# JaronTu/Multimodal_MVD_Seg

Measured on AMD Instinct MI355X. Metric: train-step samples/sec on 4-modality 128^3 patches (PlainConvUNet 3d_fullres, fp32), higher is better.
Workload: dtype f32; 1 GPU; BASELINE configs[1]: PlainConvUNet 3d_fullres 6 stages 31.2M params, 4x128x128x128 patch, 5 classes, fp32, DC+CE deep supervision, SGD-Nesterov+clip; per_gpu_batch=2, global_batch=2, parallelism=dp1, step_launch=one hipGraph replay per step (captured after 3 eager steps)

## Files before the change

include/mvdseg_hip.h:

```cpp
#ifndef MVDSEG_HIP_H
#define MVDSEG_HIP_H
#include <stddef.h>
#include <stdint.h>

#ifdef __cplusplus
extern "C" {
#endif

#define MVD_VERSION 100
#define MVD_MAX_TAPS 27

int mvd_version(void);
const char *mvd_last_error(void);
int mvd_has_mfma(void);
int mvd_set_conv_engine(int mode);
int mvd_set_wino_min_items(long n);

int mvd_pack_weight(const float *w, float *wf, float *wb, int K, int C, int T, int transposed, void *stream);

size_t mvd_conv_fwd_workspace_bytes(int N, long out_voxels, int K);
int mvd_conv3d_fwd(const float *x1, int C1, const float *x2, int C2, const float *wf, const float *bias, float *y,
                   int N, int D, int H, int W, int K, const int ksize[3], const int stride[3], void *ws,
                   size_t ws_bytes, void *stream);
int mvd_conv3d_dgrad(const float *dy, const float *wb, float *dx1, int C1, float *dx2, int C2, int N, int D, int H,
// ... 52 lines not shown
                                const int *C, const int *T, const int *transposed, void *stream);
int mvd_pack_weights_bf16_batch_pad(int n, const float *const *w, uint16_t *const *wf, uint16_t *const *wb, const int *K,
                                    const int *C, const int *T, const int *transposed, const int *Csrc, void *stream);
int mvd_conv3d_fwd_bf16(const uint16_t *x1, int C1, const uint16_t *x2, int C2, const uint16_t *wf, const float *bias,
                        uint16_t *y, int N, int D, int H, int W, int K, const int ksize[3], const int stride[3],
                        void *ws, size_t ws_bytes, void *stream);
int mvd_conv3d_dgrad_bf16(const uint16_t *dy, const uint16_t *wb, uint16_t *dx1, int C1, uint16_t *dx2, int C2, int N,
                          int D, int H, int W, int K, const int ksize[3], const int stride[3], void *ws, size_t ws_bytes,
                          void *stream);
int mvd_convT3d_fwd_bf16(const uint16_t *x, const uint16_t *wf, const float *bias, uint16_t *y, int N, int D, int H, int W,
                         int C, int K, const int stride[3], void *ws, size_t ws_bytes, void *stream);
int mvd_convT3d_dgrad_bf16(const uint16_t *dy, const uint16_t *wb, uint16_t *dx, int N, int D, int H, int W, int C, int K,
                           const int stride[3], void *ws, size_t ws_bytes, void *stream);
int mvd_conv3d_wgrad_bf16(const uint16_t *x1, int C1, const uint16_t *x2, int C2, const uint16_t *dy, float *dw,
                          float *dbias, int N, int D, int H, int W, int K, const int ksize[3], const int stride[3],
                          void *ws, size_t ws_bytes, void *stream);
int mvd_convT3d_wgrad_bf16(const uint16_t *x, const uint16_t *dy, float *dw, float *dbias, int N, int D, int H, int W,
                           int C, int K, const int stride[3], void *ws, size_t ws_bytes, void *stream);
int mvd_conv3d_fwd_bf16_stats_tiles(int N, int D, int H, int W, int C1, int C2, int K, const int ksize[3],
                                    const int stride[3]);
int mvd_conv3d_dgrad_acc_ok(int is_bf16, int N, int D, int H, int W, int C1, int K, const int ksize[3], const int stride[3]);
int mvd_conv3d_dgrad_acc(const float *dy, const float *wb, float *dx1, int C1, int N, int D, int H, int W, int K,
                         const int ksize[3], const int stride[3], void *stream);
int mvd_conv3d_dgrad_bf16_acc(const uint16_t *dy, const uint16_t *wb, uint16_t *dx1, int C1, int N, int D, int H, int W, int K,
                              const int ksize[3], const int stride[3], void *ws, size_t ws_bytes, void *stream);
int mvd_set_bf16_zmarch_kernel(int which);
int mvd_set_bf16_wgrad_kernel(int which);
int mvd_conv3d_wgrad_bf16_prologue_ok(int N, int D, int H, int W, int C1, int C2, int K, const int ksize[3], const int stride[3]);
int mvd_conv3d_wgrad_bf16_fused(const uint16_t *x1, int C1, const uint16_t *dy, float *dw, float *dbias, int N, int D, int H, int W,
                                int K, const int ksize[3], const int stride[3], const float *in_scale, const float *in_shift,
                                float slope, void *ws, size_t ws_bytes, void *stream);
int mvd_conv3d_fwd_bf16_prologue_ok(int N, int D, int H, int W, int C1, int C2, int K, const int ksize[3],
                                    const int stride[3]);
int mvd_conv3d_fwd_bf16_fused(const uint16_t *x1, int C1, const uint16_t *x2, int C2, const uint16_t *wf, const float *bias,
                              uint16_t *y, int N, int D, int H, int W, int K, const int ksize[3], const int stride[3],
                              const float *in_scale, const float *in_shift, float slope, float *tile_stats, int *ntiles_out,
                              void *ws, size_t ws_bytes, void *stream);
int mvd_instnorm_finalize_tiles(const float *tile_stats, long ntiles, const float *gamma, const float *beta, float *mean,
                                float *rstd, float *scale, float *shift, int N, long V, int C, float eps, void *stream);
int mvd_instnorm_lrelu_apply_bf16(const uint16_t *x, const float *scale, const float *shift, uint16_t *y, int N, long V,
                                  int C, float slope, void *stream);
int mvd_instnorm_stats_bf16(const void *x, int x_is_bf16, const float *gamma, const float *beta, float *mean, float *rstd,
                            float *scale, float *shift, int N, long V, int C, float eps, void *ws, size_t ws_bytes,
                            void *stream);
int mvd_instnorm_lrelu_fwd_bf16(const void *x, int x_is_bf16, const float *gamma, const float *beta, uint16_t *y,
                                float *mean, float *rstd, int N, long V, int C, float eps, float slope, void *ws,
// ... 281 lines not shown
```

multimodal_mvd_seg_amd/_lib.py:

```python
import ctypes
import os
from ctypes import c_double, c_float, c_int, c_long, c_size_t, c_uint64, c_void_p

_HERE = os.path.dirname(os.path.abspath(__file__))
LIB_PATH = os.path.join(_HERE, "libmvdseg_hip.so")

_P = c_void_p
_I3 = ctypes.c_int * 3

CONV_DIRECT, CONV_WINO2, CONV_WINO3, CONV_WINO2P = 0, 1, 2, 3

SIGNATURES = {
    "mvd_version": (c_int, []),
    "mvd_last_error": (ctypes.c_char_p, []),
    "mvd_has_mfma": (c_int, []),
    "mvd_set_conv_engine": (c_int, [c_int]),
    "mvd_set_wino_min_items": (c_int, [c_long]),
    "mvd_pack_weight": (c_int, [_P, _P, _P, c_int, c_int, c_int, c_int, _P]),
    "mvd_conv_fwd_workspace_bytes": (c_size_t, [c_int, c_long, c_int]),
    "mvd_conv3d_fwd": (c_int, [_P, c_int, _P, c_int, _P, _P, _P, c_int, c_int, c_int, c_int, c_int, _I3, _I3, _P,
                               c_size_t, _P]),
    "mvd_conv3d_dgrad": (c_int, [_P, _P, _P, c_int, _P, c_int, c_int, c_int, c_int, c_int, c_int, _I3, _I3, _P,
                                 c_size_t, _P]),
    "mvd_conv3d_wgrad_workspace_bytes": (c_size_t, [c_int, c_int, c_int, c_int, c_int, c_int, c_int]),
# ... 20 lines not shown
    "mvd_conv_wino3_applicable": (c_int, [c_int, c_int, c_int, c_int, c_int, c_int, c_int, _I3, _I3]),
    "mvd_wino3_weight_elems": (c_size_t, [c_int, c_int]),
    "mvd_pack_weight_wino3": (c_int, [_P, _P, _P, c_int, c_int, _P]),
    "mvd_pack_weights_batch3": (c_int, [c_int] + [_P] * 11 + [_P]),
    "mvd_set_wino2p_min_items": (c_int, [c_long]),
    "mvd_conv_wino2p_applicable": (c_int, [c_int, c_int, c_int, c_int, c_int, c_int, c_int, _I3, _I3]),
    "mvd_wino2p_weight_elems": (c_size_t, [c_int, c_int]),
    "mvd_pack_weight_wino2p": (c_int, [_P, _P, _P, c_int, c_int, _P]),
    "mvd_set_wgrad_wino3_min_items": (c_int, [c_long]),
    "mvd_conv_wgrad_wino3_applicable": (c_int, [c_int, c_int, c_int, c_int, c_int, c_int, c_int, _I3, _I3]),
    "mvd_wgrad_wino3_launches": (c_long, []),
    "mvd_set_wgrad_bias_fold": (c_int, [c_int]),
    "mvd_conv3d_wgrad_bf16": (c_int, [_P, c_int, _P, c_int, _P, _P, _P, c_int, c_int, c_int, c_int, c_int, _I3, _I3, _P,
                                      c_size_t, _P]),
    "mvd_convT3d_wgrad_bf16": (c_int, [_P, _P, _P, _P, c_int, c_int, c_int, c_int, c_int, c_int, _I3, _P, c_size_t,
                                       _P]),
    "mvd_instnorm_lrelu_fwd_prestats": (c_int, [_P, _P, c_long, _P, _P, _P, _P, _P, c_int, c_long, c_int, c_float, c_float,
                                                _P, c_size_t, _P]),
    "mvd_conv3d_fwd_bf16_stats_tiles": (c_int, [c_int, c_int, c_int, c_int, c_int, c_int, c_int, _I3, _I3]),
    "mvd_set_bf16_zmarch_kernel": (c_int, [c_int]),
    "mvd_set_bf16_wgrad_kernel": (c_int, [c_int]),
    "mvd_conv3d_dgrad_acc_ok": (c_int, [c_int, c_int, c_int, c_int, c_int, c_int, c_int, _I3, _I3]),
    "mvd_conv3d_dgrad_acc": (c_int, [_P, _P, _P, c_int, c_int, c_int, c_int, c_int, c_int, _I3, _I3, _P]),
    "mvd_conv3d_dgrad_bf16_acc": (c_int, [_P, _P, _P, c_int, c_int, c_int, c_int, c_int, c_int, _I3, _I3, _P, c_size_t, _P]),
    "mvd_conv3d_fwd_bf16_prologue_ok": (c_int, [c_int, c_int, c_int, c_int, c_int, c_int, c_int, _I3, _I3]),
    "mvd_conv3d_wgrad_bf16_prologue_ok": (c_int, [c_int, c_int, c_int, c_int, c_int, c_int, c_int, _I3, _I3]),
    "mvd_conv3d_wgrad_bf16_fused": (c_int, [_P, c_int, _P, _P, _P, c_int, c_int, c_int, c_int, c_int, _I3, _I3, _P, _P, c_float,
                                            _P, c_size_t, _P]),
    "mvd_instnorm_stats_bf16": (c_int, [_P, c_int, _P, _P, _P, _P, _P, _P, c_int, c_long, c_int, c_float, _P, c_size_t, _P]),
    "mvd_conv3d_fwd_bf16_fused": (c_int, [_P, c_int, _P, c_int, _P, _P, _P, c_int, c_int, c_int, c_int, c_int, _I3, _I3, _P,
                                          _P, c_float, _P, _P, _P, c_size_t, _P]),
    "mvd_instnorm_finalize_tiles": (c_int, [_P, c_long, _P, _P, _P, _P, _P, _P, c_int, c_long, c_int, c_float, _P]),
    "mvd_instnorm_lrelu_apply_bf16": (c_int, [_P, _P, _P, _P, c_int, c_long, c_int, c_float, _P]),
    "mvd_instnorm_lrelu_fwd_bf16": (c_int, [_P, c_int, _P, _P, _P, _P, _P, c_int, c_long, c_int, c_float, c_float, _P,
                                            c_size_t, _P]),
    "mvd_instnorm_lrelu_bwd_bf16": (c_int, [_P, c_int, _P, _P, _P, _P, _P, _P, _P, _P, c_int, c_long, c_int, c_float, _P,
                                            c_size_t, _P]),
    "mvd_seghead_fwd_bf16": (c_int, [_P, _P, _P, _P, c_int, c_long, c_int, c_int, _P]),
    "mvd_seghead_bwd_bf16": (c_int, [_P, _P, _P, _P, _P, _P, c_int, c_long, c_int, c_int, c_int, _P, c_size_t, _P]),
    "mvd_seghead_bf16_fused_ok": (c_int, [c_int, c_long, c_int, c_int]),
    "mvd_seghead_fwd_fused": (c_int, [_P, _P, _P, _P, _P, c_float, _P, _P, _P, c_int, c_long, c_int, c_int, _P]),
    "mvd_seghead_bwd_fused": (c_int, [_P, _P, _P, _P, _P, c_float, _P, _P, _P, _P, _P, c_int, c_long, c_int, c_int, c_int, _P,
                                      c_size_t, _P]),
    "mvd_instnorm_stats_from_tiles": (c_int, [_P, c_long, _P, _P, c_int, c_long, c_int, c_float, _P, c_size_t, _P]),
    "mvd_seghead_fwd_bf16_fused": (c_int, [_P, _P, _P, c_float, _P, _P, _P, c_int, c_long, c_int, c_int, _P]),
    "mvd_seghead_bwd_bf16_fused": (c_int, [_P, _P, _P, c_float, _P, _P, _P, _P, _P, c_int, c_long, c_int, c_int, c_int, _P,
# ... 180 lines not shown
```

multimodal_mvd_seg_amd/csrc/conv.hip:

```cpp
#include "common.h"
#include "conv_geom.h"

namespace mvd {

static int g_engine_mode = 0;
#define g_wino_off (wino_mode() == 0)
static const int g_transp_off = getenv("MVD_TRANSP") ? (atoi(getenv("MVD_TRANSP")) == 0) : 0;
static long g_wino_min_items = getenv("MVD_WINO_MIN") ? atol(getenv("MVD_WINO_MIN")) : 256;
static const long kWino3MinItemsDefault = 128;
static long g_wino3_min_items = getenv("MVD_WINO3_MIN") ? atol(getenv("MVD_WINO3_MIN")) : kWino3MinItemsDefault;
static const long kWino2pMinItemsDefault = 256;
static long g_wino2p_min_items = getenv("MVD_WINO2P_MIN") ? atol(getenv("MVD_WINO2P_MIN")) : kWino2pMinItemsDefault;

struct ConvPass {
    int N, D, H, W, R1, R2, P1, P2;
    const int *ks, *st;
};
static ConvPass fwd_pass(int N, int D, int H, int W, int C1, int C2, int K, const int ks[3], const int st[3]) {
    return {N, D, H, W, C1, C2, K, 0, ks, st};
}
static ConvPass dgrad_pass(int N, int D, int H, int W, int C1, int C2, int K, const int ks[3], const int st[3]) {
    return {N, D, H, W, K, 0, C1, C2, ks, st};
}
static bool wino_pass_ok(const ConvPass &p, int kd) {
// ... 462 lines not shown
        if (uf[q] || ub[q] || vf[q] || vb[q])
            MVD_REQUIRE((T[q] == 27 || (T[q] == 9 && !vf[q] && !vb[q])) && !transposed[q] && K[q] % 32 == 0 && C[q] % 32 == 0,
                        "pack_weights_batch3: Winograd tables need a 3x3x3 (or, uf / ub, 1x3x3) conv with C %% 32 == 0 and K %% 32 == 0");
    }
    return pack_weights_batch(n, w, wf, wb, uf, ub, K, C, T, transposed, as_stream(stream), vf, vb);
}

int mvd_set_wino2p_min_items(long n) {
    g_wino2p_min_items = n < 0 ? kWino2pMinItemsDefault : n;
    return 0;
}

size_t mvd_wino2p_weight_elems(int C, int K) { return (size_t)16 * C * K; }

int mvd_pack_weight_wino2p(const float *w, float *uf, float *ub, int K, int C, void *stream) {
    MVD_REQUIRE(w && (uf || ub) && K > 0 && C > 0, "pack_weight_wino2p: bad arguments");
    MVD_REQUIRE(K % 32 == 0 && C % 32 == 0, "pack_weight_wino2p: needs C %% 32 == 0 and K %% 32 == 0");
    return pack_weight_wino2p(w, uf, ub, K, C, as_stream(stream));
}

static bool k3s2(const int ks[3], const int st[3]) {
    return ks[0] == 3 && ks[1] == 3 && ks[2] == 3 && st[0] == 2 && st[1] == 2 && st[2] == 2;
}
static const long kDgrad32sMinVoxels = 4096;
static bool dgrad32s_eligible(int N, int D, int H, int W, int C2, const int ks[3], const int st[3]) {
    static const int dg2 = getenv("MVD_DGRAD2") ? atoi(getenv("MVD_DGRAD2")) : 1;
    if (!dg2 || g_engine_mode != 0 || C2 != 0 || !k3s2(ks, st)) return false;
    return (long)N * conv_out_dim(D, 3, 2) * conv_out_dim(H, 3, 2) * conv_out_dim(W, 3, 2) >= kDgrad32sMinVoxels || g_wino_min_items <= 1;
}

int mvd_conv3d_dgrad_routed(const float *dy, const float *wb, const float *table, int table_kind, float *dx1, int C1, float *dx2,
                            int C2, int N, int D, int H, int W, int K, const int ksize[3], const int stride[3], void *ws,
                            size_t ws_bytes, void *stream) {
    MVD_REQUIRE(dy && wb && dx1 && C1 > 0 && C2 >= 0 && (C2 == 0 || dx2), "conv3d_dgrad: null pointer / bad channels");
    MVD_REQUIRE(N > 0 && D > 0 && H > 0 && W > 0 && K > 0, "conv3d_dgrad: bad shape");
    if (check_ks(ksize, stride, "conv3d_dgrad")) return 2;
    MVD_REQUIRE(table_kind >= MVD_CONV_DIRECT && table_kind <= MVD_CONV_WINO2P, "conv3d_dgrad: unknown table kind");
    MVD_REQUIRE(!(table && table_kind == MVD_CONV_WINO2P) || (ksize[0] == 1 && ksize[1] == 3 && ksize[2] == 3),
                "conv3d_dgrad: the in-plane table is that of a 1x3x3 kernel");
    if (dgrad32s_eligible(N, D, H, W, C2, ksize, stride)) {
        int r = dgrad32s(N, D, H, W, C1, K, conv_out_dim(D, 3, 2), conv_out_dim(H, 3, 2), conv_out_dim(W, 3, 2), dy, wb, dx1,
                         as_stream(stream));
        if (r >= 0) return r;
    }
    const WinoTable tab = {table, table_kind, ksize, stride};
    for (int pd = 0; pd < stride[0]; pd++)
        for (int ph = 0; ph < stride[1]; ph++)
            for (int pw = 0; pw < stride[2]; pw++) {
                const int p[3] = {pd, ph, pw};
                FwdGeom g;
                if (!conv_dgrad_class_geom(g, N, D, H, W, C1, C2, K, ksize, stride, p)) continue;
                int r = run_fwd(g, dy, nullptr, wb, nullptr, dx1, dx2, ws, ws_bytes, as_stream(stream), &tab);
                if (r) return r;
            }
    return 0;
}

int mvd_conv3d_dgrad(const float *dy, const float *wb, float *dx1, int C1, float *dx2, int C2, int N, int D, int H, int W,
                     int K, const int ksize[3], const int stride[3], void *ws, size_t ws_bytes, void *stream) {
    return mvd_conv3d_dgrad_routed(dy, wb, nullptr, MVD_CONV_DIRECT, dx1, C1, dx2, C2, N, D, H, W, K, ksize, stride, ws, ws_bytes,
                                   stream);
}

size_t mvd_conv3d_wgrad_workspace_bytes(int C, int K, int T, int N, int Do, int Ho, int Wo) {
    WgradGeom g;
    memset(&g, 0, sizeof(g));
    g.N = N; g.Do = Do; g.Ho = Ho; g.Wo = Wo; g.C1 = C; g.C2 = 0; g.K = K; g.ntaps = g.T = T;
    size_t a = max_sz(wgrad_scalar_ws(g), wgrad_mfma_ws(g));
    return max_sz(a, colsum_ws((long)N * Do * Ho * Wo, K));
}

int mvd_set_wgrad_wino3_min_items(long n) {
    set_wgrad_wino3_min_items(n);
    return 0;
}

int mvd_conv_wgrad_wino3_applicable(int N, int D, int H, int W, int C1, int C2, int K, const int ksize[3],
// ... 206 lines not shown
                const int p[3] = {pd, ph, pw};
                FwdGeom g;
                if (!conv_dgrad_class_geom(g, N, D, H, W, C1, C2, K, ksize, stride, p)) continue;
                g.acc = (int8_t)acc;
                int r = run_fwd16(g, dy, nullptr, wb, nullptr, dx1, dx2, ws, ws_bytes, as_stream(stream));
                if (r) return r;
            }
    return 0;
}

int mvd_conv3d_dgrad_bf16(const uint16_t *dy, const uint16_t *wb, uint16_t *dx1, int C1, uint16_t *dx2, int C2, int N, int D, int H, int W,
                     int K, const int ksize[3], const int stride[3], void *ws, size_t ws_bytes, void *stream) {
    return dgrad_bf16_impl(dy, wb, dx1, C1, dx2, C2, N, D, H, W, K, ksize, stride, ws, ws_bytes, stream, 0);
}

static bool strided3(const int ksize[3], const int stride[3]) {
    return ksize[0] == 3 && ksize[1] == 3 && ksize[2] == 3 && (stride[0] == 2 || stride[1] == 2 || stride[2] == 2);
}

int mvd_conv3d_dgrad_acc_ok(int is_bf16, int N, int D, int H, int W, int C1, int K, const int ksize[3], const int stride[3]) {
    if (!conv_args_ok(N, D, H, W, C1, 0, K, ksize, stride, "conv3d_dgrad_acc_ok")) return 0;
    if (C1 % 32 || K % 32 || g_engine_mode != 0) return 0;
    if (is_bf16) return strided3(ksize, stride) ? 1 : 0;
    return (dgrad32s_eligible(N, D, H, W, 0, ksize, stride) &&
            (long)conv_out_dim(D, 3, 2) * conv_out_dim(H, 3, 2) * conv_out_dim(W, 3, 2) * K * 4 < (1L << 31)) ? 1 : 0;
}

int mvd_conv3d_dgrad_bf16_acc(const uint16_t *dy, const uint16_t *wb, uint16_t *dx1, int C1, int N, int D, int H, int W, int K,
                              const int ksize[3], const int stride[3], void *ws, size_t ws_bytes, void *stream) {
    MVD_REQUIRE(mvd_conv3d_dgrad_acc_ok(1, N, D, H, W, C1, K, ksize, stride), "conv3d_dgrad_bf16_acc: no accumulating kernel for this "
                "shape (ask mvd_conv3d_dgrad_acc_ok first)");
    return dgrad_bf16_impl(dy, wb, dx1, C1, nullptr, 0, N, D, H, W, K, ksize, stride, ws, ws_bytes, stream, 1);
}

int mvd_conv3d_dgrad_acc(const float *dy, const float *wb, float *dx1, int C1, int N, int D, int H, int W, int K,
                         const int ksize[3], const int stride[3], void *stream) {
    MVD_REQUIRE(dy && wb && dx1, "conv3d_dgrad_acc: null pointer");
    MVD_REQUIRE(mvd_conv3d_dgrad_acc_ok(0, N, D, H, W, C1, K, ksize, stride), "conv3d_dgrad_acc: no accumulating kernel for this shape "
                "(ask mvd_conv3d_dgrad_acc_ok first)");
    int r = dgrad32s(N, D, H, W, C1, K, conv_out_dim(D, 3, 2), conv_out_dim(H, 3, 2), conv_out_dim(W, 3, 2), dy, wb, dx1, as_stream(stream), 1);
    if (r < 0) {
        set_error("conv3d_dgrad_acc: the fused stride-2 kernel refused the shape");
        return 3;
    }
    return r;
}

int mvd_convT3d_fwd_bf16(const uint16_t *x, const uint16_t *wf, const float *bias, uint16_t *y, int N, int D, int H, int W, int C, int K,
                    const int stride[3], void *ws, size_t ws_bytes, void *stream) {
    MVD_REQUIRE(x && wf && y && N > 0 && D > 0 && H > 0 && W > 0 && C > 0 && K > 0, "convT3d_fwd_bf16: bad arguments");
    for (int a = 0; a < 3; a++) MVD_REQUIRE(stride[a] == 1 || stride[a] == 2, "convT3d_fwd_bf16: stride must be 1 or 2");
    if (!g_transp_off) {
        int r = convT_fwd_direct16(x, wf, bias, y, N, D, H, W, C, K, stride, as_stream(stream));
        if (r >= 0) return r;
    }
    for (int pd = 0; pd < stride[0]; pd++)
        for (int ph = 0; ph < stride[1]; ph++)
            for (int pw = 0; pw < stride[2]; pw++) {
                const int p[3] = {pd, ph, pw};
                FwdGeom g;
                convT_fwd_class_geom(g, N, D, H, W, C, K, stride, p);
                int r = run_fwd16(g, x, nullptr, wf, bias, y, nullptr, ws, ws_bytes, as_stream(stream));
                if (r) return r;
            }
    return 0;
}

int mvd_convT3d_dgrad_bf16(const uint16_t *dy, const uint16_t *wb, uint16_t *dx, int N, int D, int H, int W, int C, int K,
// ... 76 lines not shown
```

multimodal_mvd_seg_amd/csrc/conv_geom.h:

```cpp
#pragma once
#include <hip/hip_runtime.h>
#include <stdint.h>
#include <string.h>

namespace mvd {

__host__ __device__ inline int wl_ck(int C) {
    return (C % 32 == 0) ? 32 : ((C % 8 == 0) ? 8 : ((C % 4 == 0) ? 4 : 0));
}
__host__ __device__ inline size_t widx(int CK, int T, int C, int K, int t, int c, int k) {
    if (CK == 0) return ((size_t)t * C + c) * K + k;
    const int hh = CK / 2;
    const int cc = c / CK, r = c % CK;
    return ((((size_t)cc * T + t) * 2 + r / hh) * K + k) * hh + (r % hh);
}

struct FwdGeom {
    int N;
    int T;
    int Di, Hi, Wi;
    int Do, Ho, Wo;
    int Dy, Hy, Wy;
    int C1, C2, K1, K2;
    int ntaps;
// ... 167 lines not shown
size_t fwd_mfma_ws(int N, long out_vox, int K);
int fwd_mfma(const FwdGeom &g, const float *a1, const float *a2, const float *w, const float *bias, float *y1, float *y2,
             void *ws, size_t ws_bytes, hipStream_t s, float *stats = nullptr, long stats_tiles = 0, int *stats_done = nullptr,
             long *plan = nullptr);
size_t wgrad_scalar_ws(const WgradGeom &g);
int wgrad_scalar(const WgradGeom &g, const float *a1, const float *a2, const float *b, float *dw, void *ws,
                 size_t ws_bytes, hipStream_t s);
size_t wgrad_mfma_ws(const WgradGeom &g);
int wgrad_mfma(const WgradGeom &g, const float *a1, const float *a2, const float *b, float *dw, void *ws, size_t ws_bytes,
               hipStream_t s, bool bf16_in = false, float *dbias = nullptr, int *dbias_done = nullptr);

int fwd_wino(const FwdGeom &g, const float *a1, const float *a2, const float *u, const float *bias, float *y1, float *y2,
             hipStream_t s, float *stats = nullptr, int *stats_done = nullptr);
int pack_weight_wino(const float *w, float *uf, float *ub, int K, int C, hipStream_t s);
int fwd_wino3(const FwdGeom &g, const float *a1, const float *a2, const float *u, const float *bias, float *y1, float *y2,
              hipStream_t s, float *stats = nullptr, int *stats_done = nullptr);
int pack_weight_wino3(const float *w, float *uf, float *ub, int K, int C, hipStream_t s);
int wino3_enabled();
int fwd_wino2p(const FwdGeom &g, const float *a1, const float *a2, const float *u, const float *bias, float *y1, float *y2,
               hipStream_t s);
int pack_weight_wino2p(const float *w, float *uf, float *ub, int K, int C, hipStream_t s);
long wino2p_items(int N, int D, int H, int W, int K);
int dgrad32s(int N, int D, int H, int W, int C, int K, int Do, int Ho, int Wo, const float *dy, const float *wb, float *dx,
             hipStream_t s, int accumulate = 0);
int dgrad16s(int N, int D, int H, int W, int C, int K, int Do, int Ho, int Wo, const unsigned short *dy, const unsigned short *wb,
             unsigned short *dx, hipStream_t s, int accumulate = 0);
int launch_fwd16ys(const FwdGeom &g, const unsigned short *a1, const unsigned short *a2, const unsigned short *w, const float *bias,
                   unsigned short *y1, unsigned short *y2, hipStream_t s, int ncu);
int wgrad16z(const WgradGeom &g, const unsigned short *a1, const unsigned short *a2, const unsigned short *b, void *ws,
             size_t ws_bytes, bool want_bias, int *nsplit_out, float **pbias_out, hipStream_t s, const float *in_scale = nullptr,
             const float *in_shift = nullptr, float slope = 0.f);
int wgrad16z_run(const WgradGeom &g, const unsigned short *a1, const unsigned short *a2, const unsigned short *b, float *dw, void *ws,
                 size_t ws_bytes, hipStream_t s, float *dbias, int *dbias_done, const float *in_scale, const float *in_shift,
                 float slope);
bool wgrad16z_prologue_ok(const WgradGeom &g);
int wgrad16zs(const WgradGeom &g, const unsigned short *a1, const unsigned short *a2, const unsigned short *b, void *ws,
              size_t ws_bytes, int *nsplit_out, hipStream_t s);
void wgrad16z_enable(int on);
int pack_weights_batch(int n, const float *const *w, float *const *wf, float *const *wb, float *const *uf, float *const *ub,
                       const int *K, const int *C, const int *T, const int *transposed, hipStream_t s,
                       float *const *vf = nullptr, float *const *vb = nullptr);
int wino_mode();
int wgrad_wino3(const WgradGeom &g, const float *a1, const float *a2, const float *b, float *dw, void *ws, size_t ws_bytes,
                int nsplit, hipStream_t s, float *dbias, int *dbias_done);
bool wgrad_wino3_selected(const WgradGeom &g);
size_t wgrad_wino3_ws(int nsplit, int C, int K);
int wgrad_wino3_enabled();
// ... 39 lines not shown
```

multimodal_mvd_seg_amd/csrc/conv_mfma.hip:

```cpp
#include <stdlib.h>
#include <type_traits>

#include "common.h"
#include "conv_geom.h"

namespace mvd {

typedef float f32x16 __attribute__((ext_vector_type(16)));

struct FwdTile {
    int ED, EH, EW, nslots;
    int min_off[3];
    int ntd, nth, ntw;
    int K;
    int toff[27];
    int dbg;
};

__device__ __forceinline__ void store_tile32(const FwdGeom &g, const f32x16 &acc, float bv, int n, int od, int ohb, int ow0,
                                             int k, int hh, int S, int split, int Ktot, float *__restrict__ part,
                                             float *__restrict__ y1, float *__restrict__ y2) {
    const int owl = ow0 + 4 * hh;
    if (S > 1) {
        float *pl = part + (size_t)(4 * hh) * Ktot + k;
// ... 234 lines not shown
            s += p0;
            s += p1;
            s += p2;
            s += p3;
        }
        for (; j < S; j++) s += part[(size_t)j * per + idx];
        const int k = (int)(idx % K);
        size_t r = idx / K;
        const int ow = (int)(r % g.Wo);
        r /= g.Wo;
        const int oh = (int)(r % g.Ho);
        r /= g.Ho;
        const int od = (int)(r % g.Do);
        const int n = (int)(r / g.Do);
        const size_t ov = (((size_t)n * g.Dy + (od * g.so[0] + g.oo[0])) * g.Hy + (oh * g.so[1] + g.oo[1])) * g.Wy +
                          (ow * g.so[2] + g.oo[2]);
        if (k < g.K1)
            y1[ov * g.K1 + k] = s;
        else
            y2[ov * g.K2 + (k - g.K1)] = s;
    }
}

size_t fwd_mfma_ws(int N, long out_vox, int K) {
    if (out_vox > 64 * 128) return 0;
    return (size_t)MAX_SPLIT * N * out_vox * K * sizeof(float) + 256;
}

struct Fwd32Tile {
    int EH, EW, nslots;
    int magW, magHW;
    int min_off[3];
    int ntd, nth, ntw, nkb, S;
    int nitems;
    int K;
    int toff[27];
    int dbg;
};

template <int NT, int TG>
__global__ __launch_bounds__(256, 2) void k_fwd32(const FwdGeom g, const Fwd32Tile tg, const float *__restrict__ a1,
                                                  const float *__restrict__ a2, const float *__restrict__ w,
                                                  const float *__restrict__ bias, float *__restrict__ y1,
                                                  float *__restrict__ y2, float *__restrict__ part) {
    extern __shared__ __attribute__((aligned(16))) float lds[];
    constexpr int KT = 32 * NT;
    constexpr int XS = 36;
    constexpr int WS = 20;
// ... 343 lines not shown
        sa += __shfl_xor(sa, 32);
        sq += __shfl_xor(sq, 32);
        if (h == 0) *reinterpret_cast<float2 *>(so + (size_t)kcol * 2) = make_float2(sa, sq);
    }
    if (od >= g.Do) return;
#pragma unroll
    for (int r = 0; r < 16; r++) {
        const int row = (r & 3) + 8 * (r >> 2) + 4 * h;
        const int oh = oh0 + (row >> 3), ow = ow0 + (row & 7);
        if (oh < g.Ho && ow < g.Wo) {
            const size_t ov = (((size_t)n * g.Dy + od) * g.Hy + oh) * g.Wy + ow;
            const float val = acc[r] + bv;
            if (kcol < g.K1)
                y1[ov * g.K1 + kcol] = val;
            else
                y2[ov * g.K2 + (kcol - g.K1)] = val;
        }
    }
}

struct Dg2Tile {
    int ntd, nth, ntw, ncb, nitems, C;
    int acc;
};
__global__ __launch_bounds__(512, 2) void k_dgrad32s(const FwdGeom g, const Dg2Tile tg, const float *__restrict__ dy,
                                                     const float *__restrict__ wb, float *__restrict__ dx) {
    __shared__ __attribute__((aligned(16))) float Xs[135 * 36];
    constexpr int XS = 36;
    const int tid = threadIdx.x, lane = tid & 63;
    const int wave = __builtin_amdgcn_readfirstlane(tid >> 6);
    const int i = lane & 31, h = lane >> 5;
    const int per_xcd = (tg.nitems + 7) >> 3;
    const int item = (int)(blockIdx.x & 7) * per_xcd + (int)(blockIdx.x >> 3);
    if (item >= tg.nitems) return;
    unsigned r_ = (unsigned)item;
    const int cb = (int)(r_ % (unsigned)tg.ncb); r_ /= (unsigned)tg.ncb;
    const int tw_ = (int)(r_ % (unsigned)tg.ntw); r_ /= (unsigned)tg.ntw;
    const int th_ = (int)(r_ % (unsigned)tg.nth); r_ /= (unsigned)tg.nth;
    const int td_ = (int)(r_ % (unsigned)tg.ntd);
    const int n = (int)(r_ / (unsigned)tg.ntd);
    const int K = g.C1, C = tg.C;
    const int nch = K >> 5;
    const int oz0 = td_ * 2, oy0 = th_ * 4, ox0 = tw_ * 8;
    const int ccol = cb * 32 + i;
    const float *wlane = wb + (((size_t)h * C + ccol) << 4);
    const size_t wtap = (size_t)2 * C * 16;

    f32x16 acc[2];
#pragma unroll
    for (int m = 0; m < 2; m++)
#pragma unroll
        for (int r = 0; r < 16; r++) acc[m][r] = 0.f;

    for (int kk = 0; kk < nch; kk++) {
        __syncthreads();
        {
            const __amdgpu_buffer_rsrc_t rdy = __builtin_amdgcn_make_buffer_rsrc(
                const_cast<float *>(dy + (size_t)n * g.Di * g.Hi * g.Wi * K + kk * 32), 0, 0x7fffffff, 0x00020000);
            float4 v[3];
#pragma unroll
            for (int u = 0; u < 3; u++) {
                const int idx = tid + u * 512;
                const int slot = idx >> 3, part = idx & 7;
                const int ez = slot / 45, rem = slot - ez * 45;
                const int ey = rem / 9, ex = rem - ey * 9;
                const int oz = oz0 + ez, oy = oy0 + ey, ox = ox0 + ex;
                const bool ok = idx < 135 * 8 && oz < g.Di && oy < g.Hi && ox < g.Wi;
                const unsigned o = ok ? (unsigned)(((oz * g.Hi + oy) * g.Wi + ox) * K + part * 4) * 4u : 0xffffffffu;
                v[u] = __builtin_bit_cast(float4, __builtin_amdgcn_raw_buffer_load_b128(rdy, (int)o, 0, 0));
            }
#pragma unroll
            for (int u = 0; u < 3; u++) {
                const int idx = tid + u * 512;
                if (idx < 135 * 8) *reinterpret_cast<float4 *>(Xs + (size_t)(idx >> 3) * XS + (idx & 7) * 4) = v[u];
            }
        }
        __syncthreads();
// ... 21 lines not shown
                for (int u = 0; u < 2; u++) {
                    if (j + u < ntq) {
                        int t, so, tn, son;
                        tap_of(j + u, t, so);
                        tap_of(j + u + 1 < ntq ? j + u + 1 : j + u, tn, son);
#pragma unroll
                        for (int e = 0; e < 4; e++)
                            wv[(u + 1) & 1][e] = *reinterpret_cast<const float4 *>(wc + (size_t)tn * wtap + e * 4);
                        float4 af[4];
#pragma unroll
                        for (int e = 0; e < 4; e++) af[e] = xm[so * (XS / 4) + e];
#pragma unroll
                        for (int e = 0; e < 4; e++) {
                            acc[m] = __builtin_amdgcn_mfma_f32_32x32x2f32(af[e].x, wv[u][e].x, acc[m], 0, 0, 0);
                            acc[m] = __builtin_amdgcn_mfma_f32_32x32x2f32(af[e].y, wv[u][e].y, acc[m], 0, 0, 0);
                            acc[m] = __builtin_amdgcn_mfma_f32_32x32x2f32(af[e].z, wv[u][e].z, acc[m], 0, 0, 0);
                            acc[m] = __builtin_amdgcn_mfma_f32_32x32x2f32(af[e].w, wv[u][e].w, acc[m], 0, 0, 0);
                        }
                    }
                }
            }
        }
    }
    float *xl = dx + (size_t)(2 * 4 * h) * C + ccol;
#pragma unroll
    for (int m = 0; m < 2; m++) {
        const int q = m ? 7 - wave : wave;
        const int pz = q >> 2, py = (q >> 1) & 1, px = q & 1;
        const int iz = 2 * (oz0 + m) + pz;
#pragma unroll
        for (int r = 0; r < 16; r++) {
            const int iy = 2 * (oy0 + (r >> 2)) + py, ixu = 2 * (ox0 + (r & 3)) + px;
            const size_t uo = ((((size_t)n * g.Dy + iz) * g.Hy + iy) * g.Wy + ixu) * C;
            if (iz < g.Dy && iy < g.Hy && ixu + 8 * h < g.Wy) xl[uo] = tg.acc ? xl[uo] + acc[m][r] : acc[m][r];
        }
    }
}

int dgrad32s(int N, int D, int H, int W, int C, int K, int Do, int Ho, int Wo, const float *dy, const float *wb, float *dx,
             hipStream_t s, int accumulate) {
    if (C % 32 || K % 32 || (((uintptr_t)dy | (uintptr_t)wb) & 15)) return -1;
    if ((long)Do * Ho * Wo * K * 4 >= (1L << 31)) return -1;
    FwdGeom g;
    memset(&g, 0, sizeof(g));
    g.N = N;
    g.Di = Do; g.Hi = Ho; g.Wi = Wo;
    g.Dy = D; g.Hy = H; g.Wy = W;
    g.C1 = K;
    Dg2Tile tg;
    tg.ntd = (Do + 1) / 2; tg.nth = (Ho + 3) / 4; tg.ntw = (Wo + 7) / 8;
    tg.ncb = C / 32;
    tg.C = C;
    tg.acc = accumulate;
    const long nitems = (long)N * tg.ntd * tg.nth * tg.ntw * tg.ncb;
    if (nitems > (1L << 30)) return -1;
    tg.nitems = (int)nitems;
    const unsigned grid = (unsigned)(((nitems + 7) / 8) * 8);
    hipLaunchKernelGGL(k_dgrad32s, dim3(grid), dim3(512), 0, s, g, tg, dy, wb, dx);
    return check_launch("conv dgrad (stride 2, fused parity classes)");
}

static int num_cus();
static int launch_fwd32s(const FwdGeom &g, const float *a1, const float *a2, const float *w, const float *bias, float *y1,
                         float *y2, hipStream_t s, float *stats, long stats_tiles, int *stats_done, long *plan) {
    const int K = g.K1 + g.K2;
    Fwd32Tile tg;
    memset(&tg, 0, sizeof(tg));
    int mn[3] = {127, 127, 127}, mx[3] = {-127, -127, -127};
    for (int t = 0; t < g.ntaps; t++)
        for (int a = 0; a < 3; a++) {
            if (g.off[t][a] < mn[a]) mn[a] = g.off[t][a];
            if (g.off[t][a] > mx[a]) mx[a] = g.off[t][a];
        }
    const int T3[3] = {2, 4, 8};
    int E[3];
    for (int a = 0; a < 3; a++) {
        E[a] = (T3[a] - 1) * 2 + (mx[a] - mn[a]) + 1;
        tg.min_off[a] = mn[a];
    }
    tg.EH = E[1]; tg.EW = E[2];
    tg.nslots = E[0] * E[1] * E[2];
    if (tg.nslots > SXR * 64 || g.ntaps != 27) return -1;
// ... 2023 lines not shown
```

multimodal_mvd_seg_amd/ops.py:

```python
import ctypes
import os
import typing
import weakref

import numpy as np
import torch
from torch.autograd import Function
from torch.autograd.function import once_differentiable

from . import _lib
from ._lib import call, i3, query

CL3D = torch.channels_last_3d


def _stream():
    return ctypes.c_void_p(torch.cuda.current_stream().cuda_stream)


def _p(t):
    return ctypes.c_void_p(t.data_ptr()) if t is not None else None


def _require_cuda(*ts):
# ... 518 lines not shown
    @staticmethod
    @once_differentiable
    def backward(ctx, dy):
        x1, x2, wb, ub = ctx.saved_tensors
        _check_pack_generation(ctx.pack, "conv3d backward")
        _check_pack16_generation(ctx.pack16_gen, "conv3d backward")
        N, C1, C2, D, H, W, K, ks, stride, od, has_bias = ctx.geom
        dy = to_ndhwc(dy)
        dev = dy.device
        sfx = "_bf16" if ctx.bf else ""
        dx1 = dx2 = dw = db = None
        need1, need2 = ctx.needs_input_grad[0], (x2 is not None and ctx.needs_input_grad[1])
        joined = None
        if need1 and x2 is None and len(ks) == 3:
            joined = _joinable(ctx.share1, (N, C1, D, H, W), dy.dtype)
            if joined is not None and not query("mvd_conv3d_dgrad_acc_ok", int(ctx.bf), N, D, H, W, C1, K, i3(ks), i3(stride)):
                joined = None
        if joined is not None:
            if ctx.bf:
                ws = _Workspace.get(query("mvd_conv_fwd_workspace_bytes", N, D * H * W, C1), dev)
                call("mvd_conv3d_dgrad_bf16_acc", _p(dy), _p(wb), _p(joined), C1, N, D, H, W, K, i3(ks), i3(stride), _p(ws),
                     ws.numel(), _stream())
            else:
                call("mvd_conv3d_dgrad_acc", _p(dy), _p(wb), _p(joined), C1, N, D, H, W, K, i3(ks), i3(stride), _stream())
            ctx.share1.buf = None
            need1 = False
        elif need1 or need2:
            dx1 = empty_cl3d((N, C1, D, H, W), dev, dy.dtype)
            dx2 = empty_cl3d((N, C2, D, H, W), dev, dy.dtype) if x2 is not None else None
            ws = _Workspace.get(query("mvd_conv_fwd_workspace_bytes", N, D * H * W, C1 + C2), dev)
            if ctx.bf:
                call("mvd_conv3d_dgrad_bf16", _p(dy), _p(wb), _p(dx1), C1, _p(dx2), C2, N, D, H, W, K, i3(ks), i3(stride),
                     _p(ws), ws.numel(), _stream())
            else:
                call("mvd_conv3d_dgrad_routed", _p(dy), _p(wb), _p(ub), ctx.ub_kind, _p(dx1), C1, _p(dx2), C2, N, D, H, W, K,
                     i3(ks), i3(stride), _p(ws), ws.numel(), _stream())
            if need1:
                _publish(ctx.share1, dx1)
            if need2:
                _publish(ctx.share2, dx2)
        if ctx.needs_input_grad[2]:
            T = ks[0] * ks[1] * ks[2]
            weight, bias = ctx.params
            sink_w, sink_b = _take_grad(weight), (_take_grad(bias) if has_bias else None)
            dw = sink_w if sink_w is not None else torch.empty(tuple(weight.shape), dtype=torch.float32, device=dev)
            db = (sink_b if sink_b is not None else torch.empty((K,), dtype=torch.float32, device=dev)) if has_bias else None
            nb = query("mvd_conv3d_wgrad_workspace_bytes", C1 + C2, K, T, N, *od)
# ... 1627 lines not shown
```

Before: 62.64 samples/s.

## Add split-K partial-sum path to stride-2 fp32 dgrad kernel for small deep stages

The fused stride-2 dgrad kernel now splits the K-channel loop across S slices when it has few work items and the layer is small. Each slice writes a partial result into workspace, and a separate float4 reduce kernel sums the slices and optionally accumulates into dx. The minimum-voxel threshold for using this kernel is lowered so deep low-resolution stages also take it. The aim is to fill the GPU on the deep stages, at the cost of an extra launch, workspace traffic and a change in summation order.

```diff
diff --git a/include/mvdseg_hip.h b/include/mvdseg_hip.h
--- a/include/mvdseg_hip.h
+++ b/include/mvdseg_hip.h
@@ -98,6 +98,12 @@
 int mvd_conv3d_dgrad_acc_ok(int is_bf16, int N, int D, int H, int W, int C1, int K, const int ksize[3], const int stride[3]);
 int mvd_conv3d_dgrad_acc(const float *dy, const float *wb, float *dx1, int C1, int N, int D, int H, int W, int K,
                          const int ksize[3], const int stride[3], void *stream);
+int mvd_conv3d_dgrad_acc_ws(const float *dy, const float *wb, float *dx1, int C1, int N, int D, int H, int W, int K,
+                            const int ksize[3], const int stride[3], void *ws, size_t ws_bytes, void *stream);
+int mvd_dgrad32s_plan(int N, int D, int H, int W, int C, int K, size_t ws_bytes, long out[4]);
+int mvd_set_dgrad32s_min_voxels(long n);
+int mvd_set_dgrad32s_split(int s);
+long mvd_dgrad32s_launches(void);
 int mvd_conv3d_dgrad_bf16_acc(const uint16_t *dy, const uint16_t *wb, uint16_t *dx1, int C1, int N, int D, int H, int W, int K,
                               const int ksize[3], const int stride[3], void *ws, size_t ws_bytes, void *stream);
 int mvd_set_bf16_zmarch_kernel(int which);
diff --git a/multimodal_mvd_seg_amd/_lib.py b/multimodal_mvd_seg_amd/_lib.py
--- a/multimodal_mvd_seg_amd/_lib.py
+++ b/multimodal_mvd_seg_amd/_lib.py
@@ -66,6 +66,11 @@
     "mvd_set_bf16_wgrad_kernel": (c_int, [c_int]),
     "mvd_conv3d_dgrad_acc_ok": (c_int, [c_int, c_int, c_int, c_int, c_int, c_int, c_int, _I3, _I3]),
     "mvd_conv3d_dgrad_acc": (c_int, [_P, _P, _P, c_int, c_int, c_int, c_int, c_int, c_int, _I3, _I3, _P]),
+    "mvd_conv3d_dgrad_acc_ws": (c_int, [_P, _P, _P, c_int, c_int, c_int, c_int, c_int, c_int, _I3, _I3, _P, c_size_t, _P]),
+    "mvd_dgrad32s_plan": (c_int, [c_int, c_int, c_int, c_int, c_int, c_int, c_size_t, _P]),
+    "mvd_set_dgrad32s_min_voxels": (c_int, [c_long]),
+    "mvd_set_dgrad32s_split": (c_int, [c_int]),
+    "mvd_dgrad32s_launches": (c_long, []),
     "mvd_conv3d_dgrad_bf16_acc": (c_int, [_P, _P, _P, c_int, c_int, c_int, c_int, c_int, c_int, _I3, _I3, _P, c_size_t, _P]),
     "mvd_conv3d_fwd_bf16_prologue_ok": (c_int, [c_int, c_int, c_int, c_int, c_int, c_int, c_int, _I3, _I3]),
     "mvd_conv3d_wgrad_bf16_prologue_ok": (c_int, [c_int, c_int, c_int, c_int, c_int, c_int, c_int, _I3, _I3]),
diff --git a/multimodal_mvd_seg_amd/csrc/conv.hip b/multimodal_mvd_seg_amd/csrc/conv.hip
--- a/multimodal_mvd_seg_amd/csrc/conv.hip
+++ b/multimodal_mvd_seg_amd/csrc/conv.hip
@@ -508,11 +508,12 @@
 static bool k3s2(const int ks[3], const int st[3]) {
     return ks[0] == 3 && ks[1] == 3 && ks[2] == 3 && st[0] == 2 && st[1] == 2 && st[2] == 2;
 }
-static const long kDgrad32sMinVoxels = 4096;
+static const long kDgrad32sMinVoxels = 128;
+static long g_dgrad32s_min_voxels = kDgrad32sMinVoxels;
 static bool dgrad32s_eligible(int N, int D, int H, int W, int C2, const int ks[3], const int st[3]) {
     static const int dg2 = getenv("MVD_DGRAD2") ? atoi(getenv("MVD_DGRAD2")) : 1;
     if (!dg2 || g_engine_mode != 0 || C2 != 0 || !k3s2(ks, st)) return false;
-    return (long)N * conv_out_dim(D, 3, 2) * conv_out_dim(H, 3, 2) * conv_out_dim(W, 3, 2) >= kDgrad32sMinVoxels || g_wino_min_items <= 1;
+    return (long)N * conv_out_dim(D, 3, 2) * conv_out_dim(H, 3, 2) * conv_out_dim(W, 3, 2) >= g_dgrad32s_min_voxels || g_wino_min_items <= 1;
 }
 
 int mvd_conv3d_dgrad_routed(const float *dy, const float *wb, const float *table, int table_kind, float *dx1, int C1, float *dx2,
@@ -526,7 +527,7 @@
                 "conv3d_dgrad: the in-plane table is that of a 1x3x3 kernel");
     if (dgrad32s_eligible(N, D, H, W, C2, ksize, stride)) {
         int r = dgrad32s(N, D, H, W, C1, K, conv_out_dim(D, 3, 2), conv_out_dim(H, 3, 2), conv_out_dim(W, 3, 2), dy, wb, dx1,
-                         as_stream(stream));
+                         as_stream(stream), 0, ws, ws_bytes);
         if (r >= 0) return r;
     }
     const WinoTable tab = {table, table_kind, ksize, stride};
@@ -539,6 +540,28 @@
                 int r = run_fwd(g, dy, nullptr, wb, nullptr, dx1, dx2, ws, ws_bytes, as_stream(stream), &tab);
                 if (r) return r;
             }
+    return 0;
+}
+
+int mvd_set_dgrad32s_min_voxels(long n) {
+    g_dgrad32s_min_voxels = n < 0 ? kDgrad32sMinVoxels : n;
+    return 0;
+}
+
+int mvd_set_dgrad32s_split(int s) {
+    set_dgrad32s_split(s);
+    return 0;
+}
+
+long mvd_dgrad32s_launches(void) { return dgrad32s_launches(); }
+
+int mvd_dgrad32s_plan(int N, int D, int H, int W, int C, int K, size_t ws_bytes, long out[4]) {
+    const int k3[3] = {3, 3, 3}, s2[3] = {2, 2, 2};
+    long none[4];
+    if (!out) out = none;
+    const int ok = dgrad32s_plan(N, D, H, W, C, K, ws_bytes, out);
+    if (ok && N > 0 && D > 0 && H > 0 && W > 0 && dgrad32s_eligible(N, D, H, W, 0, k3, s2)) return 1;
+    out[0] = 0;
     return 0;
 }
 
@@ -791,8 +814,8 @@
     if (!conv_args_ok(N, D, H, W, C1, 0, K, ksize, stride, "conv3d_dgrad_acc_ok")) return 0;
     if (C1 % 32 || K % 32 || g_engine_mode != 0) return 0;
     if (is_bf16) return strided3(ksize, stride) ? 1 : 0;
-    return (dgrad32s_eligible(N, D, H, W, 0, ksize, stride) &&
-            (long)conv_out_dim(D, 3, 2) * conv_out_dim(H, 3, 2) * conv_out_dim(W, 3, 2) * K * 4 < (1L << 31)) ? 1 : 0;
+    long plan[4];
+    return (dgrad32s_eligible(N, D, H, W, 0, ksize, stride) && dgrad32s_plan(N, D, H, W, C1, K, 0, plan)) ? 1 : 0;
 }
 
 int mvd_conv3d_dgrad_bf16_acc(const uint16_t *dy, const uint16_t *wb, uint16_t *dx1, int C1, int N, int D, int H, int W, int K,
@@ -802,17 +825,23 @@
     return dgrad_bf16_impl(dy, wb, dx1, C1, nullptr, 0, N, D, H, W, K, ksize, stride, ws, ws_bytes, stream, 1);
 }
 
-int mvd_conv3d_dgrad_acc(const float *dy, const float *wb, float *dx1, int C1, int N, int D, int H, int W, int K,
-                         const int ksize[3], const int stride[3], void *stream) {
+int mvd_conv3d_dgrad_acc_ws(const float *dy, const float *wb, float *dx1, int C1, int N, int D, int H, int W, int K,
+                            const int ksize[3], const int stride[3], void *ws, size_t ws_bytes, void *stream) {
     MVD_REQUIRE(dy && wb && dx1, "conv3d_dgrad_acc: null pointer");
     MVD_REQUIRE(mvd_conv3d_dgrad_acc_ok(0, N, D, H, W, C1, K, ksize, stride), "conv3d_dgrad_acc: no accumulating kernel for this shape "
                 "(ask mvd_conv3d_dgrad_acc_ok first)");
-    int r = dgrad32s(N, D, H, W, C1, K, conv_out_dim(D, 3, 2), conv_out_dim(H, 3, 2), conv_out_dim(W, 3, 2), dy, wb, dx1, as_stream(stream), 1);
+    int r = dgrad32s(N, D, H, W, C1, K, conv_out_dim(D, 3, 2), conv_out_dim(H, 3, 2), conv_out_dim(W, 3, 2), dy, wb, dx1,
+                     as_stream(stream), 1, ws, ws_bytes);
     if (r < 0) {
         set_error("conv3d_dgrad_acc: the fused stride-2 kernel refused the shape");
         return 3;
     }
     return r;
+}
+
+int mvd_conv3d_dgrad_acc(const float *dy, const float *wb, float *dx1, int C1, int N, int D, int H, int W, int K,
+                         const int ksize[3], const int stride[3], void *stream) {
+    return mvd_conv3d_dgrad_acc_ws(dy, wb, dx1, C1, N, D, H, W, K, ksize, stride, nullptr, 0, stream);
 }
 
 int mvd_convT3d_fwd_bf16(const uint16_t *x, const uint16_t *wf, const float *bias, uint16_t *y, int N, int D, int H, int W, int C, int K,
diff --git a/multimodal_mvd_seg_amd/csrc/conv_geom.h b/multimodal_mvd_seg_amd/csrc/conv_geom.h
--- a/multimodal_mvd_seg_amd/csrc/conv_geom.h
+++ b/multimodal_mvd_seg_amd/csrc/conv_geom.h
@@ -213,7 +213,10 @@
 int pack_weight_wino2p(const float *w, float *uf, float *ub, int K, int C, hipStream_t s);
 long wino2p_items(int N, int D, int H, int W, int K);
 int dgrad32s(int N, int D, int H, int W, int C, int K, int Do, int Ho, int Wo, const float *dy, const float *wb, float *dx,
-             hipStream_t s, int accumulate = 0);
+             hipStream_t s, int accumulate = 0, void *ws = nullptr, size_t ws_bytes = 0);
+int dgrad32s_plan(int N, int D, int H, int W, int C, int K, size_t ws_bytes, long out[4]);
+void set_dgrad32s_split(int s);
+long dgrad32s_launches();
 int dgrad16s(int N, int D, int H, int W, int C, int K, int Do, int Ho, int Wo, const unsigned short *dy, const unsigned short *wb,
              unsigned short *dx, hipStream_t s, int accumulate = 0);
 int launch_fwd16ys(const FwdGeom &g, const unsigned short *a1, const unsigned short *a2, const unsigned short *w, const float *bias,
diff --git a/multimodal_mvd_seg_amd/csrc/conv_mfma.hip b/multimodal_mvd_seg_amd/csrc/conv_mfma.hip
--- a/multimodal_mvd_seg_amd/csrc/conv_mfma.hip
+++ b/multimodal_mvd_seg_amd/csrc/conv_mfma.hip
@@ -280,8 +280,9 @@
     }
 }
 
+static const long kSkinnyVoxels = 64 * 128;
 size_t fwd_mfma_ws(int N, long out_vox, int K) {
-    if (out_vox > 64 * 128) return 0;
+    if (out_vox > kSkinnyVoxels) return 0;
     return (size_t)MAX_SPLIT * N * out_vox * K * sizeof(float) + 256;
 }
 
@@ -671,9 +672,11 @@
 struct Dg2Tile {
     int ntd, nth, ntw, ncb, nitems, C;
     int acc;
+    int S;
 };
 __global__ __launch_bounds__(512, 2) void k_dgrad32s(const FwdGeom g, const Dg2Tile tg, const float *__restrict__ dy,
-                                                     const float *__restrict__ wb, float *__restrict__ dx) {
+                                                     const float *__restrict__ wb, float *__restrict__ dx,
+                                                     float *__restrict__ part) {
     __shared__ __attribute__((aligned(16))) float Xs[135 * 36];
     constexpr int XS = 36;
     const int tid = threadIdx.x, lane = tid & 63;
@@ -683,6 +686,7 @@
     const int item = (int)(blockIdx.x & 7) * per_xcd + (int)(blockIdx.x >> 3);
     if (item >= tg.nitems) return;
     unsigned r_ = (unsigned)item;
+    const int sp = (int)(r_ % (unsigned)tg.S); r_ /= (unsigned)tg.S;
     const int cb = (int)(r_ % (unsigned)tg.ncb); r_ /= (unsigned)tg.ncb;
     const int tw_ = (int)(r_ % (unsigned)tg.ntw); r_ /= (unsigned)tg.ntw;
     const int th_ = (int)(r_ % (unsigned)tg.nth); r_ /= (unsigned)tg.nth;
@@ -690,6 +694,8 @@
     const int n = (int)(r_ / (unsigned)tg.ntd);
     const int K = g.C1, C = tg.C;
     const int nch = K >> 5;
+    const int cbase = nch / tg.S, crem = nch - cbase * tg.S;
+    const int kk0 = sp * cbase + (sp < crem ? sp : crem), kk1 = kk0 + cbase + (sp < crem ? 1 : 0);
     const int oz0 = td_ * 2, oy0 = th_ * 4, ox0 = tw_ * 8;
     const int ccol = cb * 32 + i;
     const float *wlane = wb + (((size_t)h * C + ccol) << 4);
@@ -701,7 +707,7 @@
 #pragma unroll
         for (int r = 0; r < 16; r++) acc[m][r] = 0.f;
 
-    for (int kk = 0; kk < nch; kk++) {
+    for (int kk = kk0; kk < kk1; kk++) {
         __syncthreads();
         {
             const __amdgpu_buffer_rsrc_t rdy = __builtin_amdgcn_make_buffer_rsrc(
@@ -769,7 +775,8 @@
             }
         }
     }
-    float *xl = dx + (size_t)(2 * 4 * h) * C + ccol;
+    const bool to_part = tg.S > 1;
+    float *xl = (to_part ? part + (size_t)sp * g.N * g.Dy * g.Hy * g.Wy * C : dx) + (size_t)(2 * 4 * h) * C + ccol;
 #pragma unroll
     for (int m = 0; m < 2; m++) {
         const int q = m ? 7 - wave : wave;
@@ -779,15 +786,70 @@
         for (int r = 0; r < 16; r++) {
             const int iy = 2 * (oy0 + (r >> 2)) + py, ixu = 2 * (ox0 + (r & 3)) + px;
             const size_t uo = ((((size_t)n * g.Dy + iz) * g.Hy + iy) * g.Wy + ixu) * C;
-            if (iz < g.Dy && iy < g.Hy && ixu + 8 * h < g.Wy) xl[uo] = tg.acc ? xl[uo] + acc[m][r] : acc[m][r];
-        }
-    }
+            if (iz < g.Dy && iy < g.Hy && ixu + 8 * h < g.Wy) xl[uo] = (tg.acc && !to_part) ? xl[uo] + acc[m][r] : acc[m][r];
+        }
+    }
+}
+
+__global__ void k_dgrad32s_reduce(const float4 *__restrict__ part, float4 *__restrict__ dx, size_t per4, int S, int acc) {
+    for (size_t idx = (size_t)blockIdx.x * blockDim.x + threadIdx.x; idx < per4; idx += (size_t)gridDim.x * blockDim.x) {
+        float4 s = part[idx];
+        int j = 1;
+        for (; j + 1 < S; j += 2) {
+            const float4 p0 = part[(size_t)j * per4 + idx], p1 = part[(size_t)(j + 1) * per4 + idx];
+            s.x += p0.x; s.y += p0.y; s.z += p0.z; s.w += p0.w;
+            s.x += p1.x; s.y += p1.y; s.z += p1.z; s.w += p1.w;
+        }
+        for (; j < S; j++) {
+            const float4 p = part[(size_t)j * per4 + idx];
+            s.x += p.x; s.y += p.y; s.z += p.z; s.w += p.w;
+        }
+        if (acc) {
+            const float4 d = dx[idx];
+            s.x = d.x + s.x; s.y = d.y + s.y; s.z = d.z + s.z; s.w = d.w + s.w;
+        }
+        dx[idx] = s;
+    }
+}
+
+static int g_dgrad32s_split = 0;
+static long g_dgrad32s_launches = 0;
+void set_dgrad32s_split(int s) { g_dgrad32s_split = s > 0 ? s : 0; }
+long dgrad32s_launches() { return g_dgrad32s_launches; }
+
+static const int kDgrad32sMaxSplit = MAX_SPLIT;
+int dgrad32s_plan(int N, int D, int H, int W, int C, int K, size_t ws_bytes, long out[4]) {
+    out[0] = out[1] = out[3] = 0;
+    out[2] = 1;
+    if (N <= 0 || D <= 0 || H <= 0 || W <= 0 || C <= 0 || K <= 0 || C % 32 || K % 32) return 0;
+    const int Do = conv_out_dim(D, 3, 2), Ho = conv_out_dim(H, 3, 2), Wo = conv_out_dim(W, 3, 2);
+    if ((long)Do * Ho * Wo * K * 4 >= (1L << 31)) return 0;
+    const long items = (long)N * ((Do + 1) / 2) * ((Ho + 3) / 4) * ((Wo + 7) / 8) * (C / 32);
+    if (items > (1L << 30)) return 0;
+    const int nch = K / 32;
+    const size_t slab = (size_t)N * D * H * W * C * sizeof(float);
+    long S = 1;
+    if (g_dgrad32s_split > 0)
+        S = g_dgrad32s_split;
+    else if (items < 256 && (long)D * H * W <= kSkinnyVoxels)
+        S = 256 / items;
+    if (S > nch) S = nch;
+    if (S > kDgrad32sMaxSplit) S = kDgrad32sMaxSplit;
+    while (S > 1 && ((size_t)S * slab > ws_bytes || items * S > (1L << 30))) S--;
+    out[0] = 1;
+    out[1] = items;
+    out[2] = S;
+    out[3] = (nch + S - 1) / S;
+    return 1;
 }
 
 int dgrad32s(int N, int D, int H, int W, int C, int K, int Do, int Ho, int Wo, const float *dy, const float *wb, float *dx,
-             hipStream_t s, int accumulate) {
-    if (C % 32 || K % 32 || (((uintptr_t)dy | (uintptr_t)wb) & 15)) return -1;
-    if ((long)Do * Ho * Wo * K * 4 >= (1L << 31)) return -1;
+             hipStream_t s, int accumulate, void *ws, size_t ws_bytes) {
+    if (((uintptr_t)dy | (uintptr_t)wb) & 15) return -1;
+    const bool ws_ok = ws && !(((uintptr_t)ws | (uintptr_t)dx) & 15);
+    long plan[4];
+    if (!dgrad32s_plan(N, D, H, W, C, K, ws_ok ? ws_bytes : 0, plan)) return -1;
+    if (Do != conv_out_dim(D, 3, 2) || Ho != conv_out_dim(H, 3, 2) || Wo != conv_out_dim(W, 3, 2)) return -1;
     FwdGeom g;
     memset(&g, 0, sizeof(g));
     g.N = N;
@@ -799,12 +861,23 @@
     tg.ncb = C / 32;
     tg.C = C;
     tg.acc = accumulate;
-    const long nitems = (long)N * tg.ntd * tg.nth * tg.ntw * tg.ncb;
-    if (nitems > (1L << 30)) return -1;
+    tg.S = (int)plan[2];
+    const long nitems = plan[1] * tg.S;
     tg.nitems = (int)nitems;
     const unsigned grid = (unsigned)(((nitems + 7) / 8) * 8);
-    hipLaunchKernelGGL(k_dgrad32s, dim3(grid), dim3(512), 0, s, g, tg, dy, wb, dx);
-    return check_launch("conv dgrad (stride 2, fused parity classes)");
+    float *part = reinterpret_cast<float *>(ws);
+    hipLaunchKernelGGL(k_dgrad32s, dim3(grid), dim3(512), 0, s, g, tg, dy, wb, dx, part);
+    if (check_launch("conv dgrad (stride 2, fused parity classes)")) return 1;
+    g_dgrad32s_launches++;
+    if (tg.S > 1) {
+        const size_t per4 = (size_t)N * D * H * W * C / 4;
+        long blocks = cdiv((long)per4, 256);
+        if (blocks > 2048) blocks = 2048;
+        hipLaunchKernelGGL(k_dgrad32s_reduce, dim3((unsigned)blocks), dim3(256), 0, s, reinterpret_cast<const float4 *>(part),
+                           reinterpret_cast<float4 *>(dx), per4, tg.S, accumulate);
+        return check_launch("conv dgrad (stride 2) split reduce");
+    }
+    return 0;
 }
 
 static int num_cus();
diff --git a/multimodal_mvd_seg_amd/ops.py b/multimodal_mvd_seg_amd/ops.py
--- a/multimodal_mvd_seg_amd/ops.py
+++ b/multimodal_mvd_seg_amd/ops.py
@@ -564,7 +564,9 @@
                 call("mvd_conv3d_dgrad_bf16_acc", _p(dy), _p(wb), _p(joined), C1, N, D, H, W, K, i3(ks), i3(stride), _p(ws),
                      ws.numel(), _stream())
             else:
-                call("mvd_conv3d_dgrad_acc", _p(dy), _p(wb), _p(joined), C1, N, D, H, W, K, i3(ks), i3(stride), _stream())
+                ws = _Workspace.get(query("mvd_conv_fwd_workspace_bytes", N, D * H * W, C1), dev)
+                call("mvd_conv3d_dgrad_acc_ws", _p(dy), _p(wb), _p(joined), C1, N, D, H, W, K, i3(ks), i3(stride), _p(ws),
+                     ws.numel(), _stream())
             ctx.share1.buf = None
             need1 = False
         elif need1 or need2:
```

Result: no change. 63.08 samples/s, median of 6 (+0.7%).
